# MPEGGroup/mpeg-pcc-tmc2

Measured on AMD Instinct MI355X. Metric: encoder patch+image-gen frames/sec, longdress_vox10 32-frame GOF, higher is better.
Workload: dtype int32/f64

## Files before the change

### mpeg-pcc-tmc2_amd/csrc/api.cpp

```cpp
#include <algorithm>
#include <cstring>
#include <atomic>
#include <chrono>
#include <condition_variable>
#include <cstdarg>
#include <map>
#include <memory>
#include <mutex>

#include "internal.h"

extern char** environ;

namespace tmc2 {
int allowLargeLds( const void* kernel, size_t bytes, int device, size_t staticBytes ) {
  static std::mutex                                 lock;
  static std::map<std::pair<const void*, int>, int> granted;
  std::lock_guard<std::mutex>                       g( lock );
  int& have = granted[{kernel, device}];
  if ( int( bytes ) <= have ) return TMC2_OK;
  const int want = 160 * 1024 - int( ( staticBytes + 63 ) & ~size_t( 63 ) );
  if ( int( bytes ) > want ) {
    setError( "%zu bytes of dynamic LDS requested (+ %zu static): more than a gfx950 workgroup has", bytes, staticBytes );
    return TMC2_E_INVALID;
// ... 216 lines not shown
  tmc2_ctx* c = new tmc2_ctx();
  c->device   = device;
  hipDeviceProp_t prop;
  if ( hipGetDeviceProperties( &prop, device ) == hipSuccess ) c->cuCount = prop.multiProcessorCount;
  for ( char** e = environ; e && *e; ++e ) {
    if ( strncmp( *e, "TMC2_", 5 ) != 0 ) continue;
    const char* eq = strchr( *e, '=' );
    if ( !eq ) continue;
    c->options[std::string( *e + 5, size_t( eq - ( *e + 5 ) ) )] = std::string( eq + 1 );
  }
  if ( hipStreamCreateWithFlags( &c->stream, hipStreamNonBlocking ) != hipSuccess ) {
    setError( "hipStreamCreate failed" );
    delete c;
    return TMC2_E_HIP;
  }
  if ( hipHostMalloc( reinterpret_cast<void**>( &c->mailbox ), tmc2_ctx::kMailboxWords * 4, hipHostMallocDefault ) != hipSuccess ) {
    setError( "hipHostMalloc failed (the context's mailbox)" );
    (void)hipStreamDestroy( c->stream );
    delete c;
    return TMC2_E_HIP;
  }
  memset( c->mailbox, 0, tmc2_ctx::kMailboxWords * 4 );
  *out = c;
  return TMC2_OK;
}

int tmc2_ctx_set_option( tmc2_ctx* ctx, const char* key, const char* value ) {
  if ( !ctx || !key || !*key ) {
    tmc2::setError( "tmc2_ctx_set_option: invalid argument" );
    return TMC2_E_INVALID;
  }
  const std::string k = strncmp( key, "TMC2_", 5 ) == 0 ? key + 5 : key;
  std::lock_guard<std::mutex> g( ctx->optionsLock );
  if ( value )
    ctx->options[k] = value;
  else
    ctx->options.erase( k );
  return TMC2_OK;
}
const char* tmc2_ctx_get_option( tmc2_ctx* ctx, const char* key ) {
  if ( !ctx || !key ) return nullptr;
  const auto v = tmc2::ctxOption( ctx, strncmp( key, "TMC2_", 5 ) == 0 ? key + 5 : key );
  if ( !v ) return nullptr;
  static thread_local std::string held;
  held = *v;
  return held.c_str();
}

int tmc2_ctx_reserve( tmc2_ctx* ctx, uint64_t maxPoints, int voxelDimRefine, int bits3d, int maxCanvasWidth, int maxCanvasHeight ) {
  if ( !ctx || maxPoints == 0 || maxPoints > ( uint64_t( 1 ) << 32 ) || bits3d < 1 || bits3d > 16 || maxCanvasWidth < 0 || maxCanvasHeight < 0 ) {
    tmc2::setError( "tmc2_ctx_reserve: invalid argument" );
    return TMC2_E_INVALID;
  }
  tmc2::ApiScope scope( ctx );
  const uint64_t perPoint = voxelDimRefine > 0 && voxelDimRefine <= 2 ? 5500 : 2400;
  const int      gridShift = std::max( 1, bits3d - 1 - ( voxelDimRefine >= 4 ? 2 : ( voxelDimRefine >= 2 ? 1 : 0 ) ) );
  const uint64_t dense     = ( uint64_t( 1 ) << std::min( 33, 3 * gridShift + 1 ) ) / 32 * 8;
  const uint64_t bytes     = maxPoints * perPoint + uint64_t( maxCanvasWidth ) * uint64_t( maxCanvasHeight ) * 64 + dense + ( uint64_t( 64 ) << 20 );
  if ( !ctx->hostC.get<uint32_t>( 4 + ( size_t( maxPoints ) + 4 ) / 4 + 4 ) || !ctx->hostA.get<tmc2::OrientClusterRec>( 64 * 1024 ) ||
// ... 219 lines not shown

}

namespace tmc2 {
std::optional<std::string> ctxOption( const tmc2_ctx* ctx, const char* key ) {
  if ( !ctx ) {
    const std::string name = std::string( "TMC2_" ) + key;
    const char*       e    = getenv( name.c_str() );
    return e ? std::optional<std::string>( e ) : std::nullopt;
  }
  std::lock_guard<std::mutex> g( ctx->optionsLock );
  const auto                  it = ctx->options.find( key );
  if ( it == ctx->options.end() ) return std::nullopt;
  return it->second;
}
static std::atomic<int> g_refineOverlap{-1};
bool refineOverlap( const tmc2_ctx* ctx ) {
  if ( const auto e = ctxOption( ctx, "REFINE_OVERLAP" ) ) return ( *e )[0] == '1';
  return g_refineOverlap.load( std::memory_order_relaxed ) > 0;
}
static std::atomic<int> g_kdtreeOnHost{-1};
int kdtreePlacement( const tmc2_ctx* ctx ) {
  if ( const auto e = ctxOption( ctx, "KDTREE_HOST" ) )
    if ( ( *e )[0] >= '0' && ( *e )[0] <= '2' ) return ( *e )[0] - '0';
  const int v = g_kdtreeOnHost.load( std::memory_order_relaxed );
  return v < 0 ? 0 : v;
}
int unionPrecheck( const tmc2_ctx* ctx ) {
  const auto e = ctxOption( ctx, "UF_PRECHECK" );
  return e ? ( ( *e )[0] != '0' ) : 1;
// ... 306 lines not shown
```

### mpeg-pcc-tmc2_amd/csrc/attributes.hip

```cpp
#include <algorithm>
#include <cmath>

#include "color_transfer.h"
#include "internal.h"
#include "wave.h"
#include "patch_border_filter.h"

namespace tmc2 {
namespace {

__device__ __forceinline__ void toCanvasB( const PlaceDev& p, int u, int v, int& x, int& y ) {
  if ( p.orient == 0 ) {
    x = u + p.u0 * 16;
    y = v + p.v0 * 16;
  } else {
    x = v + p.u0 * 16;
    y = u + p.v0 * 16;
  }
}

__device__ __forceinline__ int normalCoord( const PlaceDev& p, int depth ) {
  return p.mode == 0 ? depth + p.d1 : max( 0, p.d1 - depth );
}

// ... 485 lines not shown
  StageScope       stage( ctx, "reconstruct" );
  DevBuf<uint32_t> d_tileCount, d_tileOffset, d_small;
  TMC2_TRY( d_tileCount.alloc( std::max( tiles, 1u ) ) );
  TMC2_TRY( d_tileOffset.alloc( std::max( tiles, 1u ) ) );
  TMC2_TRY( d_small.alloc( 8 ) );
  uint32_t M = 0;
  if ( tiles ) {
    if ( pbfParams )
      hipLaunchKernelGGL( ( reconTileKernel<false, true> ), dim3( tiles ), blk, 0, s, f->d_place.p, f->d_tilePatch.p, f->d_occVideo.p,
                          f->d_blockToPatch.p, f->d_geo.p, W, H, prec, d_tileCount.p, (const uint32_t*)nullptr, (Pt*)nullptr,
                          (uint32_t*)nullptr, pbf );
    else
      hipLaunchKernelGGL( reconTileKernel<false>, dim3( tiles ), blk, 0, s, f->d_place.p, f->d_tilePatch.p, f->d_occVideo.p,
                          f->d_blockToPatch.p, f->d_geo.p, W, H, prec, d_tileCount.p, (const uint32_t*)nullptr, (Pt*)nullptr,
                          (uint32_t*)nullptr, PbfMapsDev() );
    volatile uint32_t* answer = ctx->answerLine( tmc2_ctx::kAnswerRecon );
    TMC2_TRY( exclusiveScanU32( ctx, d_tileCount.p, d_tileOffset.p, tiles, d_small.p, ScanAnswer{answer, nullptr, 0} ) );
    TMC2_HIP( hipStreamSynchronize( s ) );
    M = answer[0];
  }
  if ( M == 0 && pbfParams ) {
    stage.end();
    f->reconCount         = 0;
    f->haveReconstruction = true;
    f->haveBoundaryTypes  = true;
    return TMC2_OK;
  }
  if ( M == 0 ) {
    setError( "generatePointCloud: empty reconstruction" );
    return TMC2_E_STATE;
  }
  TMC2_TRY( f->d_recon.alloc( M ) );
  TMC2_TRY( f->d_pointToPixel.alloc( M ) );
  if ( pbfParams ) {
// ... 306 lines not shown
```

### mpeg-pcc-tmc2_amd/csrc/internal.h

```cpp
#pragma once
#include <hip/hip_runtime.h>

#include <algorithm>
#include <cstdint>
#include <cstdio>
#include <cstring>
#include <initializer_list>
#include <atomic>
#include <map>
#include <memory>
#include <mutex>
#include <optional>
#include <string>
#include <functional>
#include <vector>

#include "tmc2hip.h"

namespace tmc2 {

void setError( const char* fmt, ... );

#define TMC2_HIP( expr )                                                                        \
  do {                                                                                          \
    hipError_t e_ = ( expr );                                                                   \
    if ( e_ != hipSuccess ) {                                                                   \
      tmc2::setError( "%s:%d: %s -> %s", __FILE__, __LINE__, #expr, hipGetErrorString( e_ ) ); \
      return TMC2_E_HIP;                                                                        \
    }                                                                                           \
  } while ( 0 )

// ... 228 lines not shown
  tmc2::DevBuf<unsigned long long> scanState;
  uint32_t                      scanEpoch = 0, scanTickets = 0;
  tmc2::DevBuf<uint32_t>        voxelBitmap;
  tmc2::DevBuf<uint32_t>        knnWideAdj;
  std::map<uint32_t, int>       kdLevelHint;
  struct ConstTable {
    tmc2::DevBuf<int> dev;
    std::vector<int>  host;
  };
  std::map<uint64_t, std::unique_ptr<ConstTable>> constTables;
  std::vector<std::unique_ptr<ConstTable>>        retiredTables;
  const int* constTable( uint64_t key, const std::vector<int>& host );
  uint32_t* mailbox = nullptr;
  static constexpr size_t kMailboxWords = 1024;
  volatile uint32_t* answerLine( int line ) const { return mailbox + size_t( line ) * 16; }
  enum { kAnswerRefineVoxels = 1, kAnswerPatchRound = 2, kAnswerRecon = 3, kAnswerOrientHead = 4, kAnswerTreeDepth = 5, kAnswerGeoError = 6, kAnswerAttrError = 7, kAnswerTreeLevels = 8 , kAnswerVoxelCount = 13 };
  std::map<std::string, std::string> options;
  mutable std::mutex                 optionsLock;
  std::shared_ptr<tmc2_host_gate>    hostGate;
  hipStream_t                   stream = nullptr;
  std::vector<tmc2::StageTimer> stages;
  std::vector<hipEvent_t>       freeEvents;
  bool                          timing = true;
  int                           cuCount = 256;
  void foldStage( tmc2::StageTimer& t );
  void stageAddHostMs( const char* name, double ms );

 private:
  friend struct tmc2::StageScope;
  int  stageBegin( const char* name );
  void stageEnd( int id );
// ... 199 lines not shown
bool unionCheck( const tmc2_ctx* ctx );
bool unionAgentScope( const tmc2_ctx* ctx );
int unionCheckResult( hipStream_t s, const uint32_t* d_bad, const std::string& what );
struct PassOrder {
  bool            chunked;
  const uint32_t* perm;
};
PassOrder passOrder( const tmc2_frame* f, const char* option );
int buildKdTreeDevice( tmc2_ctx* ctx, const Pt* d_pts, uint64_t n, DeviceTree& tree );
int buildKdTreePlaced( tmc2_ctx* ctx, const Pt* d_pts, uint64_t n, const int16_t* hostXyz, const char* stage, DeviceTree& tree );
int allowLargeLds( const void* kernel, size_t bytes, int device, size_t staticBytes = 64 );
struct ScanAnswer {
  volatile uint32_t* host       = nullptr;
  const uint32_t*    carry      = nullptr;
  int                carryWords = 0;
};
int exclusiveScanU32( tmc2_ctx* ctx, const uint32_t* d_in, uint32_t* d_out, size_t n, uint32_t* d_total, ScanAnswer answer = ScanAnswer() );
int radixSortPairs( tmc2_ctx* ctx, uint64_t* keyA, uint32_t* idxA, uint64_t* keyB, uint32_t* idxB, uint32_t n, uint32_t bits, bool* inA );
int markRunHeads( tmc2_ctx* ctx, const uint64_t* d_key, uint32_t n, uint32_t* d_head );
struct CellGrid;
struct MarkedCells {
  DevBuf<uint32_t> bits, rank;
  uint32_t         words = 0, count = 0;
};
int markedCells( tmc2_ctx* ctx, const Pt* d_pts, const uint8_t* d_btype, uint32_t M, const CellGrid& g, uint32_t* d_total, MarkedCells& out );
int voxelizeDevice( tmc2_ctx* ctx, const Pt* d_pts, uint32_t n, int voxDim, int maxCoord, DevBuf<Pt>& d_voxelPts, DevBuf<uint32_t>& d_voxelOfPoint,
                    uint32_t* voxelCount );
struct VoxelCloud {
  std::unique_ptr<tmc2_frame> frame;
  DevBuf<uint32_t>            d_voxelOfPoint;
  uint32_t                    count = 0;
// ... 15 lines not shown
```

### mpeg-pcc-tmc2_amd/csrc/patches.hip

```cpp
#include <algorithm>
#include <cmath>

#include "internal.h"
#include "wave.h"
#include "union_find.h"

namespace tmc2 {
namespace {

using Uf = UnionFind<false>;

constexpr uint32_t kNoLabel = 0xFFFFFFFFu;
constexpr uint32_t kFar     = 0xFFFFFFFFu;

struct PatchDev {
  int32_t u1, v1, d1;
  int32_t sizeU, sizeV, sizeU0, sizeV0;
  int32_t axN, axT, axB, mode;
  int32_t blockBase;
  int64_t depthOff;
  int64_t occOff;
};

__device__ __forceinline__ int coordOf( const Pt p, int axis ) { return axis == 0 ? p.x : ( axis == 1 ? p.y : p.z ); }
// ... 687 lines not shown
        TMC2_TRY( unionCheckResult( s, d_small.p + 8, "segmentPatches: union-find invariant broken in round " + std::to_string( rounds ) ) );
      }
      hipLaunchKernelGGL( ROUND_KERNEL( ccFlattenSeedKernel ), grd, blk, 0, s, d_raw.p, d_dist.p, thrDet, list, count, n, d_parent.p,
                          d_root.p, d_lab.p, agentScope );
    }
    uint32_t P = 0;
    for ( int guard = 0; guard < 1 << 20; ++guard ) {
      StageScope kt( ctx, "k:ccRelax" );
      for ( int b = 0; b < 3; ++b )
        hipLaunchKernelGGL( ROUND_KERNEL( ccRelaxKernel, 16 ), grd, blk, 0, s, f->d_knn.p, d_mutual.p, f->d_partition.p, d_raw.p,
                            d_root.p, perm, chunked, list, count, n, d_lab.p, d_small.p, ++relaxToken, agentScope );
      kt.end();
      hipLaunchKernelGGL( ROUND_KERNEL( ccLabelCountKernel ), grd, blk, 0, s, d_raw.p, d_root.p, d_lab.p, list, count, n, minCount,
                          d_label.p, d_ccCount.p );
      hipLaunchKernelGGL( ROUND_KERNEL( ccSeedFlagKernel ), grd, blk, 0, s, d_label.p, d_ccCount.p, minCount, list, count, d_flag.p );
      volatile uint32_t* answer = ctx->answerLine( tmc2_ctx::kAnswerPatchRound );
      TMC2_TRY( exclusiveScanU32( ctx, d_flag.p, d_rank.p, count, d_small.p + 1, ScanAnswer{answer, d_small.p, 1} ) );
      TMC2_HIP( hipStreamSynchronize( s ) );
      P = answer[0];
      if ( answer[1] != relaxToken ) break;
      if ( listed )
        hipLaunchKernelGGL( ccClearCountKernel, grd, blk, 0, s, list, count, d_ccCount.p );
      else
        TMC2_HIP( hipMemsetAsync( d_ccCount.p, 0, size_t( n ) * 4, s ) );
    }
    cc.end();
    if ( P == 0 ) break;
    StageScope build( ctx, "patches_build" );
    TMC2_TRY( d_minUv.alloc( 2 * size_t( P ) ) );
    TMC2_TRY( d_bbox.alloc( 7 * size_t( P ) ) );
    const size_t statWords = 2 * size_t( P );
    TMC2_TRY( d_patchStat.alloc( statWords ) );
    int32_t* d_view = d_bbox.p + 6 * size_t( P );
    hipLaunchKernelGGL( ROUND_KERNEL( ccAssignKernel ), grd, blk, 0, s, d_label.p, d_ccCount.p, d_rank.p, d_posOf.p, f->d_partition.p,
                        minCount, list, count, n, d_pointPatch.p, d_view );
    hipLaunchKernelGGL( patchBoundsInitKernel, dim3( ( P + 255 ) / 256 ), blk, 0, s, P, d_bbox.p, d_minUv.p, d_patchStat.p );
    if ( sp->enablePatchSplitting )
      hipLaunchKernelGGL( ROUND_KERNEL( patchMinUvKernel ), grd, blk, 0, s, f->d_pts.p, d_pointPatch.p, d_view, list, count, n,
                          d_minUv.p );
    hipLaunchKernelGGL( ROUND_KERNEL( patchTrimBboxKernel ), grd, blk, 0, s, f->d_pts.p, d_view, d_minUv.p, sp->enablePatchSplitting,
                        sp->maxPatchSize, list, count, n, d_pointPatch.p, d_bbox.p );
    int32_t* h_records = ctx->hostRecords.get<int32_t>( std::max<size_t>( 7 * size_t( P ) + statWords, size_t( 1 ) << 16 ) );
    if ( !h_records ) {
      setError( "segmentPatches: hipHostMalloc failed" );
      return TMC2_E_HIP;
    }
    const int32_t* h_bbox = h_records;
    TMC2_HIP( hipMemcpyAsync( h_records, d_bbox.p, 7 * size_t( P ) * 4, hipMemcpyDeviceToHost, s ) );
    const int32_t* h_view = h_bbox + 6 * size_t( P );
    TMC2_HIP( hipStreamSynchronize( s ) );
    for ( uint32_t p = 0; p < P; ++p )
      if ( h_bbox[6 * p] > h_bbox[6 * p + 3] ) {
        f->patches.clear();
        f->depthCount = f->occCount = 0;
        f->havePatches              = false;
        setError( "segmentPatches: patch splitting with maxPatchSize=%d keeps no point of a connected component (round %d); "
                  "the reference does not terminate on this input",
                  sp->maxPatchSize, rounds );
        return TMC2_E_UNSUPPORTED;
      }
    static const int       AX[3][3] = {{0, 2, 1}, {1, 2, 0}, {2, 0, 1}};
    std::vector<PatchDev>  h_pdLocal( P );
    PatchDev*              h_pd           = h_pdLocal.data();
    size_t                 tilesSoFar     = 0;
    const size_t           patchBase      = f->patches.size();
// ... 57 lines not shown
    TMC2_TRY( d_tables.alloc( pdBytes + size_t( tiles ) * 4 ) );
    const PatchDev* d_patches   = reinterpret_cast<const PatchDev*>( d_tables.p );
    const uint32_t* d_tilePatch = reinterpret_cast<const uint32_t*>( d_tables.p + pdBytes );
    TMC2_HIP( hipMemcpyAsync( d_tables.p, h_tables, pdBytes + size_t( tiles ) * 4, hipMemcpyHostToDevice, s ) );
    hipLaunchKernelGGL( patchInitTileKernel, dim3( tiles ), blk, 0, s, d_patches, d_tilePatch, roundDepthBase, occRes, d_map64.p );
    hipLaunchKernelGGL( ROUND_KERNEL( patchDepth0Kernel ), grd, blk, 0, s, f->d_pts.p, d_pointPatch.p, d_patches, list, count, n,
                        roundDepthBase, d_map64.p );
    hipLaunchKernelGGL( patchFilterTileKernel, dim3( tiles ), blk, 0, s, d_patches, d_tilePatch, d_map64.p, roundDepthBase, occRes,
                        sp->surfaceThickness, sp->maxAllowedDepth, d_d0tmp.p, d_d1tmp.p, d_d0src.p );
    if ( sp->surfaceThickness > 0 )
      hipLaunchKernelGGL( ROUND_KERNEL( patchDepth1Kernel ), grd, blk, 0, s, f->d_pts.p, f->d_rgb.p, d_pointPatch.p, d_patches, list,
                          count, n, roundDepthBase, sp->surfaceThickness, d_d0tmp.p, d_d0src.p, d_d1tmp.p );
    hipLaunchKernelGGL( patchResampleTileKernel, dim3( tiles ), blk, 0, s, d_patches, d_tilePatch, roundDepthBase, occRes, d_d0tmp.p,
                        d_d1tmp.p, bitmapBits, ctx->voxelBitmap.p, f->d_depth0.p, f->d_depth1.p, f->d_occupancy.p, d_patchStat.p );
    int32_t* h_stat = h_records + 7 * size_t( P );
    volatile uint32_t* answer = ctx->answerLine( tmc2_ctx::kAnswerPatchRound );
    hipLaunchKernelGGL( ROUND_KERNEL( rawDistanceKernel ), grd, blk, 0, s, f->d_pts.p, list, count, ctx->voxelBitmap.p, bitmapBits,
                        d_offsets, int( offsets.size() ), thrSel, d_dist.p, d_raw.p, d_flag.p );
    const int scanned = exclusiveScanU32( ctx, d_flag.p, d_rank.p, count, nullptr, ScanAnswer{answer, nullptr, 0} );
    if ( scanned != TMC2_OK ) {
      (void)hipStreamSynchronize( s );
      return scanned;
    }
    hipLaunchKernelGGL( ROUND_KERNEL( rawListScatterKernel ), grd, blk, 0, s, list, count, d_flag.p, d_rank.p, d_rawList[cur ^ 1].p,
                        d_posOf.p );
    TMC2_HIP( hipMemcpyAsync( h_stat, d_patchStat.p, statWords * 4, hipMemcpyDeviceToHost, s ) );
    TMC2_HIP( hipStreamSynchronize( s ) );
    const uint32_t rawBefore = rawCount;
    rawCount                 = answer[0];
    cur ^= 1;
    listed = true;
    build.end();
    if ( rawCount >= rawBefore ) {
      f->patches.clear();
      f->depthCount = f->occCount = 0;
      f->havePatches              = false;
      setError( "segmentPatches: round %d took no point off the raw list (%u left); the reference does not terminate on this input",
                rounds, rawCount );
      return TMC2_E_UNSUPPORTED;
    }
    for ( uint32_t p = 0; p < P; ++p ) {
      tmc2_patch& T = f->patches[patchBase + p];
// ... 65 lines not shown
```

### mpeg-pcc-tmc2_amd/csrc/refine.hip

```cpp
#include <algorithm>
#include <cstdlib>

#include "internal.h"
#include "wave.h"

namespace tmc2 {
namespace {

enum : uint8_t { NO_EDGE = 0x00, INDIRECT_EDGE = 0x01, M_DIRECT_EDGE = 0x10, S_DIRECT_EDGE = 0x11 };

struct Grid {
  int      voxShift, gridShift, half;
  uint32_t keyCount;
};

__device__ __forceinline__ uint32_t cellKey( int x0, int y0, int z0, int s ) {
  return uint32_t( x0 ) + ( uint32_t( y0 ) << s ) + ( uint32_t( z0 ) << ( 2 * s ) );
}

__global__ __launch_bounds__( 256 ) void voxelKeyKernel( const Pt* __restrict__ pts, uint32_t n, Grid g, uint32_t* __restrict__ key,
                                                          uint2* __restrict__ bits  ) {
  const uint32_t i = blockIdx.x * blockDim.x + threadIdx.x;
  if ( i >= n ) return;
  const Pt       p = pts[i];
// ... 907 lines not shown
  hipStream_t      s     = nullptr;
  uint32_t         n = 0, V = 0, W = 0, devStride = 32, totalLen = 0;
  int              devRange = 1, idBits = 26;
  Grid             g{};
  std::vector<int> rows;
  uint2*           bits       = nullptr;
  bool             bitsFilled = false;
  int              capTier = 2;
  size_t           Vp = 0, W2 = 0, ball = 0, perVoxel = 0;
  uint64_t         capacity = 0;
  uint32_t         res[5] = {0, 0, 0, 0, 0};
  uint32_t         hitRegionCap = 0;
  DevBuf<uint32_t> d_key, d_flag, d_vid, d_small, d_count, d_rowLen, d_devLen, d_adjOff, d_hist, d_activeBuf, d_pointStart,
      d_pointList, d_cursor, d_lastRescore, d_flags, d_gbits, d_adj, d_dev, d_lastKey, d_roffG, d_rlenG, d_radjG,
      d_voxelOfRank, d_hitBuf, d_hitCtl, d_hitOff, d_hitLen, d_rowCtl;
  std::vector<uint32_t> rowCtlHost;
  DevBuf<Pt>      d_centre;
  DevBuf<double>  d_weight;
  DevBuf<uint8_t> d_state;
  const int*      d_rows = nullptr;
  bool matches( int nn, double l, int it, int vd, int sr ) const {
    return nn == maxNNCount && l == lambda && it == iterationCount && vd == voxDim && sr == searchRadius;
  }
  uint64_t rowTableEntries( size_t perVoxel ) const {
    const uint64_t groups = ( uint64_t( V ) + 15 ) / 16, perRegion = 16 * ( ( groups + kRowRegions - 1 ) / kRowRegions );
    return uint64_t( kRowRegions ) * perRegion * perVoxel;
  }
  int  geometry( tmc2_frame* f );
  int  finish();
  void launchNeighbourhood();
  ~RefineJob();
// ... 26 lines not shown
  hipLaunchKernelGGL( ( neighbourhoodKernel<CAP, WAVES> ), dim3( ( V + WAVES - 1 ) / WAVES ), dim3( 64 * WAVES ), 0, s, d_centre.p,      \
                      d_count.p, g, V, d_rows, nRows, maxNNCount, lambda, idBits, devRange, devStride,                      \
                      rowRegionCap, d_rowLen.p, d_devLen.p, d_weight.p, d_adjOff.p, d_adj.p, d_dev.p, d_rowCtl.p,            \
                      d_small.p + 2, bits, reinterpret_cast<const uint2*>( d_voxelOfRank.p ), d_lastKey.p, savedHits );      \
  hipLaunchKernelGGL( ( reverseRowsKernel<CAP, WAVES> ), dim3( ( V + WAVES - 1 ) / WAVES ), dim3( 64 * WAVES ), 0, s, d_centre.p, reinterpret_cast<const uint2*>( d_voxelOfRank.p ), \
                      bits, g, V, d_rows, nRows, idBits, d_lastKey.p, rowRegionCap, d_roffG.p, d_rlenG.p, d_radjG.p,          \
                      d_rowCtl.p + kRowRegions * 32, d_small.p + 2, savedHits )
  switch ( capTier ) {
    case 0: TMC2_NEIGHBOURHOOD( 1024, 8 ); break;
    case 1: TMC2_NEIGHBOURHOOD( 1280, 4 ); break;
    case 2: TMC2_NEIGHBOURHOOD( 1536, 4 ); break;
    case 3: TMC2_NEIGHBOURHOOD( 2048, 4 ); break;
    default: TMC2_NEIGHBOURHOOD( 4096, 2 ); break;
  }
#undef TMC2_NEIGHBOURHOOD
}

int RefineJob::geometry( tmc2_frame* f ) {
  if ( voxDim < 2 || ( voxDim & ( voxDim - 1 ) ) ) {
    setError( "refineSegmentationGridBased: voxelDimensionRefineSegmentation=%d unsupported (power of two >= 2)", voxDim );
    return TMC2_E_UNSUPPORTED;
  }
  if ( iterationCount < 1 ) iterationCount = 1;
  frame = f;
  ctx   = f->ctx;
  s     = ctx->stream;
  n     = uint32_t( f->n );
  size_t geoRange = 1;
  for ( size_t i = size_t( f->geoMax - 1 ); i != 0; i >>= 1, geoRange <<= 1 ) {}
  g.voxShift = 0;
// ... 51 lines not shown
    const uint32_t   words  = g.keyCount / 32 + 2;
    const uint32_t   blocks = ( words + kBitsBlock - 1 ) / kBitsBlock;
    DevBuf<uint32_t> d_blockTotal, d_blockBase;
    TMC2_TRY( d_blockTotal.alloc( blocks ) );
    TMC2_TRY( d_blockBase.alloc( blocks ) );
    TMC2_TRY( d_firstPoint.alloc( n ) );
    TMC2_HIP( hipMemsetAsync( d_firstPoint.p, 0xFF, size_t( n ) * 4, s ) );
    hipLaunchKernelGGL( bitsBlockCountKernel, dim3( blocks ), blk, 0, s, bits, words, d_blockTotal.p );
    TMC2_TRY( exclusiveScanU32( ctx, d_blockTotal.p, d_blockBase.p, blocks, nullptr ) );
    hipLaunchKernelGGL( bitsPrefixKernel, dim3( blocks ), blk, 0, s, bits, words, d_blockBase.p );
    hipLaunchKernelGGL( firstPointKernel, grdN, blk, 0, s, d_key.p, n, bits, d_firstPoint.p );
  }
  hipLaunchKernelGGL( firstFlagKernel, grdN, blk, 0, s, d_key.p, bits, d_firstPoint.p, n, d_flag.p );
  DevBuf<uint32_t> d_rank;
  TMC2_TRY( d_rank.alloc( n ) );
  volatile uint32_t* answer = ctx->answerLine( tmc2_ctx::kAnswerRefineVoxels );
  TMC2_TRY( exclusiveScanU32( ctx, d_flag.p, d_rank.p, n, d_small.p, ScanAnswer{answer, nullptr, 0} ) );
  TMC2_HIP( hipStreamSynchronize( s ) );
  V = answer[0];
  TMC2_TRY( d_count.alloc( size_t( V ) + 1 ) );
  TMC2_TRY( d_rowLen.alloc( V ) );
  TMC2_TRY( d_devLen.alloc( V ) );
  TMC2_TRY( d_adjOff.alloc( V + 1 ) );
  TMC2_TRY( d_hist.alloc( size_t( V ) * 4 ) );
  TMC2_TRY( d_centre.alloc( V ) );
  TMC2_TRY( d_weight.alloc( V ) );
  Vp = ( size_t( V ) + 63 ) & ~size_t( 63 );
  TMC2_TRY( d_state.alloc( Vp * 2 ) );
  TMC2_TRY( d_activeBuf.alloc( V ) );
  W = ( V + 31 ) / 32;
  W2          = ( size_t( V ) + 15 ) / 16;
  const size_t closureZeroWords = 2 * W2 + 2 * size_t( kSubLists ) * 32 + 64;
  TMC2_TRY( d_pointStart.alloc( size_t( V ) + 1 ) );
  TMC2_TRY( d_pointList.alloc( n ) );
// ... 41 lines not shown
  TMC2_TRY( d_radjG.alloc( size_t( capacity ) ) );
  {
    const auto   hitsEnv = ctxOption( ctx, "REFINE_HITS" );
    const size_t perHit  = hitsEnv && ( *hitsEnv )[0] == 't' ? 1 : std::min<size_t>( ball, size_t( ctx->refineHitsPerVoxel ) );
    if ( uint64_t( V ) * perHit < 0xFFFFFFFFull ) {
      hitRegionCap = uint32_t( ( uint64_t( V ) * perHit + kHitRegions - 1 ) / kHitRegions );
      TMC2_TRY( d_hitBuf.alloc( size_t( hitRegionCap ) * kHitRegions ) );
      TMC2_TRY( d_hitCtl.alloc( kHitRegions * 32 ) );
      TMC2_TRY( d_hitOff.alloc( V ) );
      TMC2_TRY( d_hitLen.alloc( V ) );
      TMC2_TRY( fillRegions( ctx, {{d_hitCtl.p, kHitRegions * 32 * 4, 0}} ) );
    }
  }
  TMC2_TRY( d_rowCtl.alloc( 2 * kRowRegions * 32 ) );
  TMC2_TRY( fillRegions( ctx, {{d_rowCtl.p, 2 * kRowRegions * 32 * 4, 0}} ) );
  rowCtlHost.assign( kRowRegions * 32, 0u );
  launchNeighbourhood();
  TMC2_HIP( hipMemcpyAsync( res, d_small.p + 1, 20, hipMemcpyDeviceToHost, s ) );
  TMC2_HIP( hipMemcpyAsync( rowCtlHost.data(), d_rowCtl.p, kRowRegions * 32 * 4, hipMemcpyDeviceToHost, s ) );
  TMC2_HIP( hipGetLastError() );
  return TMC2_OK;
}

int RefineJob::finish() {
  tmc2_frame* f = frame;
  if ( !f->haveNormals || !f->havePartition ) {
    setError( "refineSegmentationGridBased: normals / partition missing" );
    return TMC2_E_STATE;
  }
  StageScope setup( ctx, "refine_setup" );
  const dim3 blk( 256 ), grdN( ( n + 255 ) / 256 );
  uint8_t *d_edge = d_state.p, *d_ppi = d_state.p + Vp;
  uint32_t* d_active = d_activeBuf.p;
  const dim3 grdV( ( V + 255 ) / 256 ), grdV16( ( V + 15 ) / 16 );
  for ( int attempt = 0;; ++attempt ) {
    TMC2_HIP( hipStreamSynchronize( s ) );
    TMC2_HIP( hipGetLastError() );
    totalLen = 0;
    for ( uint32_t r = 0; r < kRowRegions; ++r ) totalLen += rowCtlHost[r * 32];
    if ( ctxOption( ctx, "REFINE_DEBUG" ) ) fprintf( stderr, "refine: neighbourhood attempt %d tier %d: %u row entries, overflow word %u (V = %u)\n", attempt, capTier, totalLen, res[1], V );
    if ( res[4] ) {
      ctx->refineHitsPerVoxel = std::min<uint32_t>( 4096u - 160u, ctx->refineHitsPerVoxel * 7u / 4u );
      ctx->stageAddHostMs( "refine_hits_out_of_room", 0.0 );
    }
    if ( res[1] == 0 ) break;
    if ( ( res[1] != 1 && res[1] != 3 ) || attempt > 3 || ( res[1] == 3 && capTier >= kLastCapTier ) ) {
      setError( "refineSegmentationGridBased: neighbourhood pass failed (%u)", res[1] );
      return TMC2_E_HIP;
    }
    if ( res[1] == 3 ) {
      capTier            = std::max( capTier + 1, capTierFor( res[3] ) );
      ctx->refineCapTier = capTier;
      ctx->stageAddHostMs( "refine_cap_tier_repeat", 0.0 );
    } else {
      perVoxel = ball;
    }
    capacity = rowTableEntries( perVoxel );
    if ( capacity > 0xFFFFFFFFull ) {
      setError( "refineSegmentationGridBased: %u voxels x %zu row entries exceed the neighbourhood table", V, perVoxel );
      return TMC2_E_UNSUPPORTED;
    }
    TMC2_TRY( d_adj.alloc( size_t( capacity ) ) );
    TMC2_TRY( d_radjG.alloc( size_t( capacity ) ) );
    TMC2_HIP( hipMemsetAsync( d_small.p + 1, 0, 20, s ) );
    if ( d_hitCtl.p ) TMC2_HIP( hipMemsetAsync( d_hitCtl.p, 0, kHitRegions * 32 * 4, s ) );
    TMC2_HIP( hipMemsetAsync( d_rowCtl.p, 0, 2 * kRowRegions * 32 * 4, s ) );
    launchNeighbourhood();
    TMC2_HIP( hipMemcpyAsync( res, d_small.p + 1, 20, hipMemcpyDeviceToHost, s ) );
    TMC2_HIP( hipMemcpyAsync( rowCtlHost.data(), d_rowCtl.p, kRowRegions * 32 * 4, hipMemcpyDeviceToHost, s ) );
  }
  d_hitBuf.release(), d_hitCtl.release(), d_hitOff.release(), d_hitLen.release();
  hipLaunchKernelGGL( bitsCleanKernel, grdN, blk, 0, s, d_key.p, n, bits );
  bitsFilled = false;
  hipLaunchKernelGGL( histAccumulateKernel, grdN, blk, 0, s, d_vid.p, f->d_partition.p, (const uint8_t*)nullptr, n,
                      d_hist.p );
  hipLaunchKernelGGL( initVoxelStateKernel, grdV, blk, 0, s, reinterpret_cast<const uint4*>( d_hist.p ), d_count.p, V,
                      d_edge, d_ppi, d_active );
  DevBuf<uint32_t> d_lists;
  DevBuf<uint4>    d_rec;
  TMC2_TRY( d_lists.alloc( size_t( kSubLists ) * V ) );
  TMC2_TRY( d_rec.alloc( 2 * size_t( V ) ) );
  hipLaunchKernelGGL( smoothInitKernel, grdV16, blk, 0, s, reinterpret_cast<const uint4*>( d_hist.p ), d_adjOff.p,
                      d_rowLen.p, d_adj.p, V, d_rec.p );
  setup.end();
// ... 103 lines not shown
```

### mpeg-pcc-tmc2_amd/csrc/scan.hip

```cpp
#include <algorithm>

#include "internal.h"
#include "wave.h"

namespace tmc2 {
namespace {
constexpr int kTile = 2048;

constexpr unsigned long long kAggregate = 1ull << 32, kInclusive = 2ull << 32;
__global__ __launch_bounds__( 256 ) void scanLookBackKernel( const uint32_t* __restrict__ in, uint32_t* __restrict__ out,
                                                              uint32_t n, unsigned long long* __restrict__ state,
                                                              uint32_t epoch, uint32_t ticketBase, uint32_t tiles,
                                                              uint32_t* __restrict__ total, ScanAnswer answer ) {
  __shared__ uint32_t waveTotal[4];
  __shared__ uint32_t sTile, sPrefix;
  if ( threadIdx.x == 0 ) sTile = atomicAdd( reinterpret_cast<uint32_t*>( state ), 1u ) - ticketBase;
  __syncthreads();
  const uint32_t tile = sTile;
  const int      lane = threadIdx.x & 63, wave = threadIdx.x >> 6;
  const uint32_t base = tile * kTile + threadIdx.x * 8;
  uint32_t       v[8], run = 0;
#pragma unroll
  for ( int k = 0; k < 8; ++k ) {
    v[k] = ( base + k < n ) ? in[base + k] : 0u;
// ... 17 lines not shown
        }
        const unsigned long long running = __ballot( ( ( w >> 32 ) & 3u ) == 2u );
        const int                first   = running ? __ffsll( static_cast<long long>( running ) ) - 1 : 64;
        prefix += waveSum( lane <= first ? static_cast<uint32_t>( w ) : 0u );
        if ( running ) break;
        j -= 64;
      }
      if ( lane == 0 )
        __hip_atomic_store( &st[tile], tag | kInclusive | ( prefix + aggregate ), __ATOMIC_RELAXED, __HIP_MEMORY_SCOPE_AGENT );
    }
    if ( lane == 0 ) {
      sPrefix = prefix;
      if ( tile + 1 == tiles ) {
        if ( total ) *total = prefix + aggregate;
        if ( answer.host ) {
          answer.host[0] = prefix + aggregate;
          for ( int k = 0; k < answer.carryWords; ++k ) answer.host[1 + k] = answer.carry[k];
        }
      }
    }
  }
  __syncthreads();
  offset += sPrefix;
#pragma unroll
  for ( int k = 0; k < 8; ++k ) {
    if ( base + k < n ) out[base + k] = offset;
    offset += v[k];
  }
}

constexpr int    kFillMax   = 12;
constexpr size_t kFillBlock = 16384;
struct FillArgs {
  unsigned long long base[kFillMax], bytes[kFillMax];
  uint32_t           firstBlock[kFillMax + 1], word[kFillMax];
  int                count;
};
__global__ __launch_bounds__( 256 ) void fillRegionsKernel( const FillArgs a ) {
  int r = 0;
  while ( r + 1 < a.count && blockIdx.x >= a.firstBlock[r + 1] ) ++r;
  uint8_t* const p     = reinterpret_cast<uint8_t*>( a.base[r] );
  const size_t   head  = reinterpret_cast<size_t>( p ) & 15, end = head + a.bytes[r];
  uint8_t* const line0 = p - head;
// ... 34 lines not shown
    ctx->scanEpoch   = 1;
    ctx->scanTickets = 0;
  }
  hipLaunchKernelGGL( scanLookBackKernel, dim3( tiles ), dim3( 256 ), 0, ctx->stream, d_in, d_out, uint32_t( n ),
                      ctx->scanState.p, ctx->scanEpoch, ctx->scanTickets, tiles, d_total, answer );
  const hipError_t launched = hipGetLastError();
  if ( launched != hipSuccess ) {
    ctx->scanState.release();
    setError( "exclusiveScanU32: %s", hipGetErrorString( launched ) );
    return TMC2_E_HIP;
  }
  ctx->scanTickets += tiles;
  return TMC2_OK;
}

int fillRegions( tmc2_ctx* ctx, std::initializer_list<FillRegion> regions ) {
  FillArgs a{};
  uint32_t blocks = 0;
  for ( const FillRegion& r : regions ) {
    if ( r.bytes == 0 ) continue;
    if ( a.count == kFillMax ) {
      setError( "fillRegions: more than %d regions", kFillMax );
      return TMC2_E_INVALID;
    }
    a.base[a.count]       = reinterpret_cast<unsigned long long>( r.p );
    a.bytes[a.count]      = r.bytes;
    a.word[a.count]       = r.value * 0x01010101u;
    a.firstBlock[a.count] = blocks;
    blocks += uint32_t( ( ( reinterpret_cast<size_t>( r.p ) & 15 ) + r.bytes + kFillBlock - 1 ) / kFillBlock );
    ++a.count;
// ... 11 lines not shown
```

Measured before the change: 197.2.

## Replace stream synchronizations with token-published host answer lines and spin polling

GPU kernels now write their answer words with system-scope atomic stores into a coherent pinned mailbox, then publish a per-call sequence token. The host spin-polls for that token for a bounded time and falls back to hipStreamSynchronize only if the bound expires. Small device-to-host copies (patch bboxes, patch stats, refine row counts) move from hipMemcpyAsync to a one-block publish kernel that writes straight into pinned host memory. The aim is to cut the latency of the blocking syncs in the patch segmentation, refine and reconstruction loops. The cost is busy-waiting CPU time, and coherent (uncached) host memory for the mailbox.

```diff
diff --git a/mpeg-pcc-tmc2_amd/csrc/answer_wait.h b/mpeg-pcc-tmc2_amd/csrc/answer_wait.h
--- /dev/null
+++ b/mpeg-pcc-tmc2_amd/csrc/answer_wait.h
@@ -0,0 +1,50 @@
+#pragma once
+#include <chrono>
+#include <cstdint>
+#if defined( __x86_64__ ) || defined( __i386__ )
+#include <immintrin.h>
+#endif
+
+namespace tmc2 {
+constexpr int kAnswerTokenWord = 15;
+
+struct AnswerSeq {
+  uint32_t last = 0;
+  uint32_t next() {
+    if ( ++last == 0 ) ++last;
+    return last;
+  }
+};
+struct AnswerTicket {
+  volatile uint32_t* line  = nullptr;
+  uint32_t           token = 0;
+};
+inline AnswerTicket answerArm( volatile uint32_t* line, AnswerSeq& seq ) {
+  __atomic_store_n( line + kAnswerTokenWord, 0u, __ATOMIC_RELAXED );
+  return AnswerTicket{line, seq.next()};
+}
+inline bool answerArrived( const AnswerTicket& t ) { return __atomic_load_n( t.line + kAnswerTokenWord, __ATOMIC_ACQUIRE ) == t.token; }
+inline void answerPause() {
+#if defined( __x86_64__ ) || defined( __i386__ )
+  _mm_pause();
+#endif
+}
+inline bool answerPoll( const AnswerTicket& t, uint64_t boundNs ) {
+  if ( boundNs == 0 ) return false;
+  const auto t0 = std::chrono::steady_clock::now();
+  for ( ;; ) {
+    for ( int spin = 0; spin < 16; ++spin ) {
+      if ( answerArrived( t ) ) return true;
+      answerPause();
+    }
+    if ( uint64_t( std::chrono::duration_cast<std::chrono::nanoseconds>( std::chrono::steady_clock::now() - t0 ).count() ) >= boundNs ) return false;
+  }
+}
+enum class AnswerEnd { Polled, FellBack, DrainFailed, Lost  };
+template <typename Drain>
+inline AnswerEnd answerWait( const AnswerTicket& t, uint64_t boundNs, Drain&& drain ) {
+  if ( answerPoll( t, boundNs ) ) return AnswerEnd::Polled;
+  if ( !drain() ) return AnswerEnd::DrainFailed;
+  return answerArrived( t ) ? AnswerEnd::FellBack : AnswerEnd::Lost;
+}
+}
diff --git a/mpeg-pcc-tmc2_amd/csrc/api.cpp b/mpeg-pcc-tmc2_amd/csrc/api.cpp
--- a/mpeg-pcc-tmc2_amd/csrc/api.cpp
+++ b/mpeg-pcc-tmc2_amd/csrc/api.cpp
@@ -254,7 +254,7 @@
     delete c;
     return TMC2_E_HIP;
   }
-  if ( hipHostMalloc( reinterpret_cast<void**>( &c->mailbox ), tmc2_ctx::kMailboxWords * 4, hipHostMallocDefault ) != hipSuccess ) {
+  if ( hipHostMalloc( reinterpret_cast<void**>( &c->mailbox ), tmc2_ctx::kMailboxWords * 4, hipHostMallocCoherent ) != hipSuccess ) {
     setError( "hipHostMalloc failed (the context's mailbox)" );
     (void)hipStreamDestroy( c->stream );
     delete c;
@@ -280,9 +280,17 @@
 }
 const char* tmc2_ctx_get_option( tmc2_ctx* ctx, const char* key ) {
   if ( !ctx || !key ) return nullptr;
+  static thread_local std::string held;
+  if ( strcmp( strncmp( key, "TMC2_", 5 ) == 0 ? key + 5 : key, "ANSWER_WAITS" ) == 0 ) {
+    char buf[160];
+    snprintf( buf, sizeof( buf ), "%llu %llu %llu %llu %llu %llu", (unsigned long long)ctx->answerWaits[0].load(), (unsigned long long)ctx->answerWaits[1].load(),
+              (unsigned long long)ctx->answerWaits[2].load(), (unsigned long long)ctx->answerWaitUs[0].load(), (unsigned long long)ctx->answerWaitUs[1].load(),
+              (unsigned long long)ctx->answerWaitUs[2].load() );
+    held = buf;
+    return held.c_str();
+  }
   const auto v = tmc2::ctxOption( ctx, strncmp( key, "TMC2_", 5 ) == 0 ? key + 5 : key );
   if ( !v ) return nullptr;
-  static thread_local std::string held;
   held = *v;
   return held.c_str();
 }
@@ -532,6 +540,32 @@
   if ( it == ctx->options.end() ) return std::nullopt;
   return it->second;
 }
+int waitAnswer( tmc2_ctx* ctx, const AnswerTicket& ticket, const char* who ) {
+  const auto t0       = std::chrono::steady_clock::now();
+  const auto count    = [&]( int how ) {
+    ctx->answerWaits[how].fetch_add( 1, std::memory_order_relaxed );
+    ctx->answerWaitUs[how].fetch_add( uint64_t( std::chrono::duration_cast<std::chrono::microseconds>( std::chrono::steady_clock::now() - t0 ).count() ), std::memory_order_relaxed );
+    return TMC2_OK;
+  };
+  const auto syncOpt  = ctxOption( ctx, "ANSWER_SYNC" );
+  const bool sync     = syncOpt && ( *syncOpt )[0] == '1';
+  uint64_t   boundUs  = ctx->answerPollUs;
+  if ( const auto b = ctxOption( ctx, "ANSWER_POLL_US" ) ) boundUs = strtoull( b->c_str(), nullptr, 10 );
+  int        failed = TMC2_OK;
+  const auto drain  = [&]() -> int {
+    TMC2_HIP( hipStreamSynchronize( ctx->stream ) );
+    TMC2_HIP( hipGetLastError() );
+    return TMC2_OK;
+  };
+  switch ( answerWait( ticket, sync ? 0 : std::min<uint64_t>( boundUs, 3600ull * 1000 * 1000 ) * 1000, [&] { return ( failed = drain() ) == TMC2_OK; } ) ) {
+    case AnswerEnd::Polled: return count( 0 );
+    case AnswerEnd::FellBack: return count( sync ? 2 : 1 );
+    case AnswerEnd::DrainFailed: return failed;
+    default: break;
+  }
+  setError( "%s: the stream drained without the token of its answer line", who );
+  return TMC2_E_HIP;
+}
 static std::atomic<int> g_refineOverlap{-1};
 bool refineOverlap( const tmc2_ctx* ctx ) {
   if ( const auto e = ctxOption( ctx, "REFINE_OVERLAP" ) ) return ( *e )[0] == '1';
diff --git a/mpeg-pcc-tmc2_amd/csrc/attributes.hip b/mpeg-pcc-tmc2_amd/csrc/attributes.hip
--- a/mpeg-pcc-tmc2_amd/csrc/attributes.hip
+++ b/mpeg-pcc-tmc2_amd/csrc/attributes.hip
@@ -523,10 +523,10 @@
       hipLaunchKernelGGL( reconTileKernel<false>, dim3( tiles ), blk, 0, s, f->d_place.p, f->d_tilePatch.p, f->d_occVideo.p,
                           f->d_blockToPatch.p, f->d_geo.p, W, H, prec, d_tileCount.p, (const uint32_t*)nullptr, (Pt*)nullptr,
                           (uint32_t*)nullptr, PbfMapsDev() );
-    volatile uint32_t* answer = ctx->answerLine( tmc2_ctx::kAnswerRecon );
-    TMC2_TRY( exclusiveScanU32( ctx, d_tileCount.p, d_tileOffset.p, tiles, d_small.p, ScanAnswer{answer, nullptr, 0} ) );
-    TMC2_HIP( hipStreamSynchronize( s ) );
-    M = answer[0];
+    const AnswerTicket points = ctx->armAnswer( tmc2_ctx::kAnswerRecon );
+    TMC2_TRY( exclusiveScanU32( ctx, d_tileCount.p, d_tileOffset.p, tiles, d_small.p, ScanAnswer{points.line, nullptr, 0, points.token} ) );
+    TMC2_TRY( waitAnswer( ctx, points, "generatePointCloud" ) );
+    M = points.line[0];
   }
   if ( M == 0 && pbfParams ) {
     stage.end();
diff --git a/mpeg-pcc-tmc2_amd/csrc/internal.h b/mpeg-pcc-tmc2_amd/csrc/internal.h
--- a/mpeg-pcc-tmc2_amd/csrc/internal.h
+++ b/mpeg-pcc-tmc2_amd/csrc/internal.h
@@ -15,6 +15,7 @@
 #include <functional>
 #include <vector>
 
+#include "answer_wait.h"
 #include "tmc2hip.h"
 
 namespace tmc2 {
@@ -273,7 +274,11 @@
   uint32_t* mailbox = nullptr;
   static constexpr size_t kMailboxWords = 1024;
   volatile uint32_t* answerLine( int line ) const { return mailbox + size_t( line ) * 16; }
-  enum { kAnswerRefineVoxels = 1, kAnswerPatchRound = 2, kAnswerRecon = 3, kAnswerOrientHead = 4, kAnswerTreeDepth = 5, kAnswerGeoError = 6, kAnswerAttrError = 7, kAnswerTreeLevels = 8 , kAnswerVoxelCount = 13 };
+  tmc2::AnswerSeq    answerSeq;
+  uint32_t           answerPollUs = 400;
+  std::atomic<uint64_t> answerWaits[3] = {}, answerWaitUs[3] = {};
+  tmc2::AnswerTicket armAnswer( int line ) { return tmc2::answerArm( answerLine( line ), answerSeq ); }
+  enum { kAnswerRefineVoxels = 1, kAnswerPatchRound = 2, kAnswerRecon = 3, kAnswerOrientHead = 4, kAnswerTreeDepth = 5, kAnswerGeoError = 6, kAnswerAttrError = 7, kAnswerTreeLevels = 8 , kAnswerVoxelCount = 13, kAnswerRefineRows = 16  };
   std::map<std::string, std::string> options;
   mutable std::mutex                 optionsLock;
   std::shared_ptr<tmc2_host_gate>    hostGate;
@@ -503,7 +508,19 @@
   volatile uint32_t* host       = nullptr;
   const uint32_t*    carry      = nullptr;
   int                carryWords = 0;
-};
+  uint32_t           token      = 0;
+};
+int waitAnswer( tmc2_ctx* ctx, const AnswerTicket& ticket, const char* who );
+int publishWords( tmc2_ctx* ctx, const uint32_t* d_src, size_t words, volatile uint32_t* hostDst, const AnswerTicket& ticket );
+#if defined( __HIPCC__ )
+__device__ inline void answerStore( volatile uint32_t* p, uint32_t v ) {
+  __hip_atomic_store( const_cast<uint32_t*>( p ), v, __ATOMIC_RELAXED, __HIP_MEMORY_SCOPE_SYSTEM );
+}
+__device__ inline void answerPublish( volatile uint32_t* line, uint32_t token ) {
+  __threadfence_system();
+  answerStore( line + kAnswerTokenWord, token );
+}
+#endif
 int exclusiveScanU32( tmc2_ctx* ctx, const uint32_t* d_in, uint32_t* d_out, size_t n, uint32_t* d_total, ScanAnswer answer = ScanAnswer() );
 int radixSortPairs( tmc2_ctx* ctx, uint64_t* keyA, uint32_t* idxA, uint64_t* keyB, uint32_t* idxB, uint32_t n, uint32_t bits, bool* inA );
 int markRunHeads( tmc2_ctx* ctx, const uint64_t* d_key, uint32_t n, uint32_t* d_head );
diff --git a/mpeg-pcc-tmc2_amd/csrc/patches.hip b/mpeg-pcc-tmc2_amd/csrc/patches.hip
--- a/mpeg-pcc-tmc2_amd/csrc/patches.hip
+++ b/mpeg-pcc-tmc2_amd/csrc/patches.hip
@@ -725,11 +725,11 @@
       hipLaunchKernelGGL( ROUND_KERNEL( ccLabelCountKernel ), grd, blk, 0, s, d_raw.p, d_root.p, d_lab.p, list, count, n, minCount,
                           d_label.p, d_ccCount.p );
       hipLaunchKernelGGL( ROUND_KERNEL( ccSeedFlagKernel ), grd, blk, 0, s, d_label.p, d_ccCount.p, minCount, list, count, d_flag.p );
-      volatile uint32_t* answer = ctx->answerLine( tmc2_ctx::kAnswerPatchRound );
-      TMC2_TRY( exclusiveScanU32( ctx, d_flag.p, d_rank.p, count, d_small.p + 1, ScanAnswer{answer, d_small.p, 1} ) );
-      TMC2_HIP( hipStreamSynchronize( s ) );
-      P = answer[0];
-      if ( answer[1] != relaxToken ) break;
+      const AnswerTicket seeds = ctx->armAnswer( tmc2_ctx::kAnswerPatchRound );
+      TMC2_TRY( exclusiveScanU32( ctx, d_flag.p, d_rank.p, count, d_small.p + 1, ScanAnswer{seeds.line, d_small.p, 1, seeds.token} ) );
+      TMC2_TRY( waitAnswer( ctx, seeds, "segmentPatches" ) );
+      P = seeds.line[0];
+      if ( seeds.line[1] != relaxToken ) break;
       if ( listed )
         hipLaunchKernelGGL( ccClearCountKernel, grd, blk, 0, s, list, count, d_ccCount.p );
       else
@@ -757,9 +757,10 @@
       return TMC2_E_HIP;
     }
     const int32_t* h_bbox = h_records;
-    TMC2_HIP( hipMemcpyAsync( h_records, d_bbox.p, 7 * size_t( P ) * 4, hipMemcpyDeviceToHost, s ) );
+    const AnswerTicket boxes = ctx->armAnswer( tmc2_ctx::kAnswerPatchRound );
+    TMC2_TRY( publishWords( ctx, reinterpret_cast<const uint32_t*>( d_bbox.p ), 7 * size_t( P ), reinterpret_cast<volatile uint32_t*>( h_records ), boxes ) );
     const int32_t* h_view = h_bbox + 6 * size_t( P );
-    TMC2_HIP( hipStreamSynchronize( s ) );
+    TMC2_TRY( waitAnswer( ctx, boxes, "segmentPatches" ) );
     for ( uint32_t p = 0; p < P; ++p )
       if ( h_bbox[6 * p] > h_bbox[6 * p + 3] ) {
         f->patches.clear();
@@ -847,7 +848,8 @@
     hipLaunchKernelGGL( patchResampleTileKernel, dim3( tiles ), blk, 0, s, d_patches, d_tilePatch, roundDepthBase, occRes, d_d0tmp.p,
                         d_d1tmp.p, bitmapBits, ctx->voxelBitmap.p, f->d_depth0.p, f->d_depth1.p, f->d_occupancy.p, d_patchStat.p );
     int32_t* h_stat = h_records + 7 * size_t( P );
-    volatile uint32_t* answer = ctx->answerLine( tmc2_ctx::kAnswerPatchRound );
+    const AnswerTicket rawLeft = ctx->armAnswer( tmc2_ctx::kAnswerPatchRound );
+    volatile uint32_t* answer  = rawLeft.line;
     hipLaunchKernelGGL( ROUND_KERNEL( rawDistanceKernel ), grd, blk, 0, s, f->d_pts.p, list, count, ctx->voxelBitmap.p, bitmapBits,
                         d_offsets, int( offsets.size() ), thrSel, d_dist.p, d_raw.p, d_flag.p );
     const int scanned = exclusiveScanU32( ctx, d_flag.p, d_rank.p, count, nullptr, ScanAnswer{answer, nullptr, 0} );
@@ -857,8 +859,12 @@
     }
     hipLaunchKernelGGL( ROUND_KERNEL( rawListScatterKernel ), grd, blk, 0, s, list, count, d_flag.p, d_rank.p, d_rawList[cur ^ 1].p,
                         d_posOf.p );
-    TMC2_HIP( hipMemcpyAsync( h_stat, d_patchStat.p, statWords * 4, hipMemcpyDeviceToHost, s ) );
-    TMC2_HIP( hipStreamSynchronize( s ) );
+    const int published = publishWords( ctx, reinterpret_cast<const uint32_t*>( d_patchStat.p ), statWords, reinterpret_cast<volatile uint32_t*>( h_stat ), rawLeft );
+    if ( published != TMC2_OK ) {
+      (void)hipStreamSynchronize( s );
+      return published;
+    }
+    TMC2_TRY( waitAnswer( ctx, rawLeft, "segmentPatches" ) );
     const uint32_t rawBefore = rawCount;
     rawCount                 = answer[0];
     cur ^= 1;
diff --git a/mpeg-pcc-tmc2_amd/csrc/refine.hip b/mpeg-pcc-tmc2_amd/csrc/refine.hip
--- a/mpeg-pcc-tmc2_amd/csrc/refine.hip
+++ b/mpeg-pcc-tmc2_amd/csrc/refine.hip
@@ -945,7 +945,9 @@
   DevBuf<uint32_t> d_key, d_flag, d_vid, d_small, d_count, d_rowLen, d_devLen, d_adjOff, d_hist, d_activeBuf, d_pointStart,
       d_pointList, d_cursor, d_lastRescore, d_flags, d_gbits, d_adj, d_dev, d_lastKey, d_roffG, d_rlenG, d_radjG,
       d_voxelOfRank, d_hitBuf, d_hitCtl, d_hitOff, d_hitLen, d_rowCtl;
-  std::vector<uint32_t> rowCtlHost;
+  AnswerTicket     rowsTicket;
+  int              publishNeighbourhoodAnswer();
+  int              awaitNeighbourhoodAnswer();
   DevBuf<Pt>      d_centre;
   DevBuf<double>  d_weight;
   DevBuf<uint8_t> d_state;
@@ -1002,6 +1004,29 @@
     default: TMC2_NEIGHBOURHOOD( 4096, 2 ); break;
   }
 #undef TMC2_NEIGHBOURHOOD
+}
+
+__global__ __launch_bounds__( 128 ) void neighbourhoodAnswerKernel( const uint32_t* __restrict__ small, const uint32_t* __restrict__ rowCtl,
+                                                                     volatile uint32_t* line, uint32_t token ) {
+  static_assert( kRowRegions == 128, "one thread per region" );
+  if ( threadIdx.x < 5 ) answerStore( line + threadIdx.x, small[1 + threadIdx.x] );
+  answerStore( line + 16 + threadIdx.x, rowCtl[threadIdx.x * 32] );
+  __threadfence_system();
+  __syncthreads();
+  if ( threadIdx.x == 0 ) answerPublish( line, token );
+}
+int RefineJob::publishNeighbourhoodAnswer() {
+  rowsTicket = ctx->armAnswer( tmc2_ctx::kAnswerRefineRows );
+  hipLaunchKernelGGL( neighbourhoodAnswerKernel, dim3( 1 ), dim3( 128 ), 0, s, d_small.p, d_rowCtl.p, rowsTicket.line, rowsTicket.token );
+  TMC2_HIP( hipGetLastError() );
+  return TMC2_OK;
+}
+int RefineJob::awaitNeighbourhoodAnswer() {
+  TMC2_TRY( waitAnswer( ctx, rowsTicket, "refineSegmentationGridBased" ) );
+  for ( int k = 0; k < 5; ++k ) res[k] = rowsTicket.line[k];
+  totalLen = 0;
+  for ( uint32_t r = 0; r < kRowRegions; ++r ) totalLen += rowsTicket.line[16 + r];
+  return TMC2_OK;
 }
 
 int RefineJob::geometry( tmc2_frame* f ) {
@@ -1083,10 +1108,10 @@
   hipLaunchKernelGGL( firstFlagKernel, grdN, blk, 0, s, d_key.p, bits, d_firstPoint.p, n, d_flag.p );
   DevBuf<uint32_t> d_rank;
   TMC2_TRY( d_rank.alloc( n ) );
-  volatile uint32_t* answer = ctx->answerLine( tmc2_ctx::kAnswerRefineVoxels );
-  TMC2_TRY( exclusiveScanU32( ctx, d_flag.p, d_rank.p, n, d_small.p, ScanAnswer{answer, nullptr, 0} ) );
-  TMC2_HIP( hipStreamSynchronize( s ) );
-  V = answer[0];
+  const AnswerTicket voxels = ctx->armAnswer( tmc2_ctx::kAnswerRefineVoxels );
+  TMC2_TRY( exclusiveScanU32( ctx, d_flag.p, d_rank.p, n, d_small.p, ScanAnswer{voxels.line, nullptr, 0, voxels.token} ) );
+  TMC2_TRY( waitAnswer( ctx, voxels, "refineSegmentationGridBased" ) );
+  V = voxels.line[0];
   TMC2_TRY( d_count.alloc( size_t( V ) + 1 ) );
   TMC2_TRY( d_rowLen.alloc( V ) );
   TMC2_TRY( d_devLen.alloc( V ) );
@@ -1158,11 +1183,8 @@
   }
   TMC2_TRY( d_rowCtl.alloc( 2 * kRowRegions * 32 ) );
   TMC2_TRY( fillRegions( ctx, {{d_rowCtl.p, 2 * kRowRegions * 32 * 4, 0}} ) );
-  rowCtlHost.assign( kRowRegions * 32, 0u );
   launchNeighbourhood();
-  TMC2_HIP( hipMemcpyAsync( res, d_small.p + 1, 20, hipMemcpyDeviceToHost, s ) );
-  TMC2_HIP( hipMemcpyAsync( rowCtlHost.data(), d_rowCtl.p, kRowRegions * 32 * 4, hipMemcpyDeviceToHost, s ) );
-  TMC2_HIP( hipGetLastError() );
+  TMC2_TRY( publishNeighbourhoodAnswer() );
   return TMC2_OK;
 }
 
@@ -1178,10 +1200,7 @@
   uint32_t* d_active = d_activeBuf.p;
   const dim3 grdV( ( V + 255 ) / 256 ), grdV16( ( V + 15 ) / 16 );
   for ( int attempt = 0;; ++attempt ) {
-    TMC2_HIP( hipStreamSynchronize( s ) );
-    TMC2_HIP( hipGetLastError() );
-    totalLen = 0;
-    for ( uint32_t r = 0; r < kRowRegions; ++r ) totalLen += rowCtlHost[r * 32];
+    TMC2_TRY( awaitNeighbourhoodAnswer() );
     if ( ctxOption( ctx, "REFINE_DEBUG" ) ) fprintf( stderr, "refine: neighbourhood attempt %d tier %d: %u row entries, overflow word %u (V = %u)\n", attempt, capTier, totalLen, res[1], V );
     if ( res[4] ) {
       ctx->refineHitsPerVoxel = std::min<uint32_t>( 4096u - 160u, ctx->refineHitsPerVoxel * 7u / 4u );
@@ -1210,8 +1229,7 @@
     if ( d_hitCtl.p ) TMC2_HIP( hipMemsetAsync( d_hitCtl.p, 0, kHitRegions * 32 * 4, s ) );
     TMC2_HIP( hipMemsetAsync( d_rowCtl.p, 0, 2 * kRowRegions * 32 * 4, s ) );
     launchNeighbourhood();
-    TMC2_HIP( hipMemcpyAsync( res, d_small.p + 1, 20, hipMemcpyDeviceToHost, s ) );
-    TMC2_HIP( hipMemcpyAsync( rowCtlHost.data(), d_rowCtl.p, kRowRegions * 32 * 4, hipMemcpyDeviceToHost, s ) );
+    TMC2_TRY( publishNeighbourhoodAnswer() );
   }
   d_hitBuf.release(), d_hitCtl.release(), d_hitOff.release(), d_hitLen.release();
   hipLaunchKernelGGL( bitsCleanKernel, grdN, blk, 0, s, d_key.p, n, bits );
diff --git a/mpeg-pcc-tmc2_amd/csrc/scan.hip b/mpeg-pcc-tmc2_amd/csrc/scan.hip
--- a/mpeg-pcc-tmc2_amd/csrc/scan.hip
+++ b/mpeg-pcc-tmc2_amd/csrc/scan.hip
@@ -55,8 +55,9 @@
       if ( tile + 1 == tiles ) {
         if ( total ) *total = prefix + aggregate;
         if ( answer.host ) {
-          answer.host[0] = prefix + aggregate;
-          for ( int k = 0; k < answer.carryWords; ++k ) answer.host[1 + k] = answer.carry[k];
+          answerStore( answer.host, prefix + aggregate );
+          for ( int k = 0; k < answer.carryWords; ++k ) answerStore( answer.host + 1 + k, answer.carry[k] );
+          if ( answer.token ) answerPublish( answer.host, answer.token );
         }
       }
     }
@@ -68,6 +69,14 @@
     if ( base + k < n ) out[base + k] = offset;
     offset += v[k];
   }
+}
+
+__global__ __launch_bounds__( 256 ) void publishWordsKernel( const uint32_t* __restrict__ src, uint32_t words, volatile uint32_t* hostDst,
+                                                              volatile uint32_t* line, uint32_t token ) {
+  for ( uint32_t i = threadIdx.x; i < words; i += 256 ) answerStore( hostDst + i, src[i] );
+  __threadfence_system();
+  __syncthreads();
+  if ( threadIdx.x == 0 ) answerPublish( line, token );
 }
 
 constexpr int    kFillMax   = 12;
@@ -132,6 +141,16 @@
   return TMC2_OK;
 }
 
+int publishWords( tmc2_ctx* ctx, const uint32_t* d_src, size_t words, volatile uint32_t* hostDst, const AnswerTicket& ticket ) {
+  if ( words > 0xFFFFFFFFull || !ticket.line || !ticket.token || ( words && ( !d_src || !hostDst ) ) ) {
+    setError( "publishWords: invalid argument" );
+    return TMC2_E_INVALID;
+  }
+  hipLaunchKernelGGL( publishWordsKernel, dim3( 1 ), dim3( 256 ), 0, ctx->stream, d_src, uint32_t( words ), hostDst, ticket.line, ticket.token );
+  TMC2_HIP( hipGetLastError() );
+  return TMC2_OK;
+}
+
 int fillRegions( tmc2_ctx* ctx, std::initializer_list<FillRegion> regions ) {
   FillArgs a{};
   uint32_t blocks = 0;
```

Result: no change. 197.3 (median of 2 runs) (+0.0%).
